# Scalsol/mega.pytorch

Measured on AMD Instinct MI355X. Metric: frames/sec MEGA R-101 inference, 1000x600 VID clip, higher is better.
Workload: dtype bf16

## Files before the change

### mega/pytorch_amd/csrc/bneck64.hip

```cpp
#include <cstdlib>

#include "common.h"

namespace {

constexpr int BK_TY = 8, BK_TX = 16;
constexpr int BK_PY = BK_TY + 2, BK_PX = BK_TX + 2;
constexpr int BK_NP = BK_PY * BK_PX;
constexpr int BK_M1 = 192;
constexpr int BK_NT = 512;
constexpr int BK_W2ROW = 1168;
constexpr int BK_WROW = 144;
constexpr int BK_SBROW = 528;
constexpr int BK_OFF_W2 = 0;
constexpr int BK_OFF_T1 = 64 * BK_W2ROW;
constexpr int BK_OFF_XB = BK_OFF_T1 + BK_NP * 128;
constexpr int BK_OFF_W1 = BK_OFF_XB + BK_M1 * 128;
constexpr int BK_XB_BYTES = 256 * BK_WROW;
constexpr int BK_OFF_T2 = BK_OFF_XB + BK_XB_BYTES;
constexpr int BK_LDS = BK_OFF_T2 + 128 * 128;
constexpr int BK_OFF_ST = BK_OFF_T1;
static_assert(BK_OFF_ST + 128 * BK_SBROW <= BK_LDS, "staging must fit");
static_assert(BK_M1 * 128 + 64 * BK_WROW <= BK_XB_BYTES, "x chunk + w1 chunk must fit the XB region");

struct Bneck64Params {
  const bf16_t* x;
  const bf16_t* w1;
  const bf16_t* w2;
  const bf16_t* w3;
  const float *s1, *b1, *s2, *b2, *s3, *b3;
  bf16_t* out;
  int N, H, W, tiles_y, tiles_x, ntiles;
};

template <typename HT>
__device__ __forceinline__ f32x16_t bk_mma(f32x16_t acc, const uint4& a, const uint4& b) {
  return Half16<HT>::mfma32(__builtin_bit_cast(u32x4_t, a), __builtin_bit_cast(u32x4_t, b), acc);
}

template <typename HT>
__device__ __forceinline__ unsigned bk_relu_pack(float a, float b) {
  const s16x2_t z = {0, 0};
  return __builtin_bit_cast(unsigned, __builtin_elementwise_max(__builtin_bit_cast(s16x2_t, Half16<HT>::pack2(a, b)), z));
}
template <typename HT>
__device__ __forceinline__ bf16_t bk_relu1(float a) {
  const bf16_t h = Half16<HT>::cvt(a);
  return (short)h < 0 ? (bf16_t)0 : h;
}

template <typename HT>
__global__ __launch_bounds__(BK_NT, 2) void bneck64_kernel(Bneck64Params p) {
  extern __shared__ __attribute__((aligned(16))) unsigned char smem[];
  unsigned char* const w2l = smem + BK_OFF_W2;
  unsigned char* const t1l = smem + BK_OFF_T1;
  unsigned char* const xbl = smem + BK_OFF_XB;
  unsigned char* const w1l = smem + BK_OFF_W1;
  unsigned char* const t2l = smem + BK_OFF_T2;
  unsigned char* const sbl = smem + BK_OFF_ST;
  const int tid = threadIdx.x, lane = tid & 63, wave = tid >> 6;
  const int l31 = lane & 31, h = lane >> 5;

  {
    const uint4* wg = reinterpret_cast<const uint4*>(p.w2);
    for (int e = tid; e < 64 * 72; e += BK_NT) {
      const int n = e / 72, c = e - n * 72;
      *reinterpret_cast<uint4*>(w2l + n * BK_W2ROW + c * 16) = wg[e];
    }
  }

  const unsigned xbytes = (unsigned)((size_t)p.N * p.H * p.W * 512);
  const __amdgpu_buffer_rsrc_t rs_x = __builtin_amdgcn_make_buffer_rsrc(const_cast<bf16_t*>(p.x), 0, (int)xbytes, 0x00020000);
  const __amdgpu_buffer_rsrc_t rs_o = __builtin_amdgcn_make_buffer_rsrc(p.out, 0, (int)xbytes, 0x00020000);
  constexpr unsigned OOB = 0x80000000u;

  auto tile_origin = [&](int t, int& n, int& y0, int& x0) {
    const int per_img = p.tiles_y * p.tiles_x;
    n = t / per_img;
    const int r = t - n * per_img;
    const int ty = r / p.tiles_x;
    y0 = ty * BK_TY;
    x0 = (r - ty * p.tiles_x) * BK_TX;
  };

  u32x4_t px[12], pw1[4];
  auto prefetch = [&](int t) {
    int n, y0, x0;
    const bool live = t < p.ntiles;
    tile_origin(live ? t : 0, n, y0, x0);
    unsigned off[3];
#pragma unroll
    for (int i = 0; i < 3; ++i) {
      const int v = tid + BK_NT * i;
      const int row = v >> 3, j = v & 7;
      const int py = row / BK_PX, pxx = row - py * BK_PX;
      const int yy = y0 - 1 + py, xx = x0 - 1 + pxx;
      const bool ok = live && row < BK_NP && (unsigned)yy < (unsigned)p.H && (unsigned)xx < (unsigned)p.W;
      off[i] = ok ? (unsigned)(((n * p.H + yy) * p.W + xx) * 512 + j * 16) : OOB;
    }
#pragma unroll
    for (int kc = 0; kc < 4; ++kc) {
#pragma unroll
      for (int i = 0; i < 3; ++i) {
        px[3 * kc + i] = __builtin_amdgcn_raw_buffer_load_b128(rs_x, off[i], kc * 128, 0);
      }
      pw1[kc] = *reinterpret_cast<const u32x4_t*>(p.w1 + (tid >> 3) * 256 + kc * 64 + (tid & 7) * 8);
    }
  };

  const int r1 = 32 * wave + l31;
  const unsigned a1_base = (unsigned)(r1 * 128), a1_sw = (unsigned)((r1 >> 1) & 7);
  const unsigned b1_base = (unsigned)(l31 * BK_WROW + h * 16);
  const int mb2 = wave >> 1, nb2 = wave & 1;
  const int ay = 2 * mb2 + (l31 >> 4), ax = l31 & 15;
  const unsigned a2_base = (unsigned)((ay * BK_PX + ax) * 128);
  const int b2_off = (32 * nb2 + l31) * BK_W2ROW + h * 16;
  const unsigned a3_base = (unsigned)(l31 * 128), a3_sw = (unsigned)((l31 >> 1) & 7);
  const unsigned b3_base = (unsigned)((32 * wave + l31) * BK_WROW + h * 16);
  const float s1a = p.s1[l31], s1b = p.s1[32 + l31], b1a = p.b1[l31], b1b = p.b1[32 + l31];
  const float s2v = p.s2[32 * nb2 + l31], b2v = p.b2[32 * nb2 + l31];
  const float s3v = p.s3[32 * wave + l31], b3v = p.b3[32 * wave + l31];

  int t = blockIdx.x;
  prefetch(t);
  __syncthreads();
  for (; t < p.ntiles; t += gridDim.x) {
    int n, y0, x0;
    tile_origin(t, n, y0, x0);
    f32x16_t c1a, c1b;
#pragma unroll
    for (int r = 0; r < 16; ++r) { c1a[r] = 0.f; c1b[r] = 0.f; }
#pragma unroll
    for (int kc = 0; kc < 4; ++kc) {
#pragma unroll
      for (int i = 0; i < 3; ++i) {
        const int v = tid + BK_NT * i;
        const int row = v >> 3, j = v & 7;
        *reinterpret_cast<u32x4_t*>(xbl + row * 128 + ((j ^ ((row >> 1) & 7)) * 16)) = px[3 * kc + i];
      }
      *reinterpret_cast<u32x4_t*>(w1l + (tid >> 3) * BK_WROW + (tid & 7) * 16) = pw1[kc];
      __syncthreads();
      if (wave < 6) {
#pragma unroll
        for (int ks = 0; ks < 4; ++ks) {
          const uint4 a = *reinterpret_cast<const uint4*>(xbl + a1_base + (((unsigned)(2 * ks + h) ^ a1_sw) << 4));
          const uint4 b0 = *reinterpret_cast<const uint4*>(w1l + b1_base + ks * 32);
          const uint4 b1 = *reinterpret_cast<const uint4*>(w1l + 32 * BK_WROW + b1_base + ks * 32);
          c1a = bk_mma<HT>(c1a, a, b0);
          c1b = bk_mma<HT>(c1b, a, b1);
        }
      }
      __syncthreads();
    }
    u32x4_t pw3[4];
#pragma unroll
    for (int i = 0; i < 4; ++i) pw3[i] = reinterpret_cast<const u32x4_t*>(p.w3)[tid + BK_NT * i];
    int ho = h, lo = l31;
    asm volatile("" : "+v"(ho), "+v"(lo));
    if (wave < 6) {
#pragma unroll
      for (int r = 0; r < 16; ++r) {
        const int R = 32 * wave + (r & 3) + 8 * (r >> 2) + 4 * ho;
        if (R < BK_NP) {
          const int py = R / BK_PX, pxx = R - py * BK_PX;
          const int yy = y0 - 1 + py, xx = x0 - 1 + pxx;
          const bool in = (unsigned)yy < (unsigned)p.H && (unsigned)xx < (unsigned)p.W;
          const bf16_t ra = bk_relu1<HT>(c1a[r] * s1a + b1a), rb = bk_relu1<HT>(c1b[r] * s1b + b1b);
          const bf16_t va = in ? ra : (bf16_t)0;
          const bf16_t vb = in ? rb : (bf16_t)0;
          unsigned char* base = t1l + R * 128;
          const int sw = (pxx >> 1) & 7;
          *reinterpret_cast<bf16_t*>(base + (((lo >> 3) ^ sw) * 16) + (lo & 7) * 2) = va;
          *reinterpret_cast<bf16_t*>(base + ((((32 + lo) >> 3) ^ sw) * 16) + (lo & 7) * 2) = vb;
        }
      }
    }
#pragma unroll
    for (int i = 0; i < 4; ++i) {
      const int v = tid + BK_NT * i;
      *reinterpret_cast<u32x4_t*>(xbl + (v >> 3) * BK_WROW + (v & 7) * 16) = pw3[i];
    }
    prefetch(t + gridDim.x);
    __syncthreads();
    f32x16_t c2;
#pragma unroll
    for (int r = 0; r < 16; ++r) c2[r] = 0.f;
#pragma unroll
    for (int kh = 0; kh < 3; ++kh)
#pragma unroll
      for (int kw = 0; kw < 3; ++kw)
#pragma unroll
        for (int ks = 0; ks < 4; ++ks) {
          const unsigned sw2 = (unsigned)(((ax + kw) >> 1) & 7);
          const uint4 a = *reinterpret_cast<const uint4*>(t1l + a2_base + (kh * BK_PX + kw) * 128 +
                                                          (((unsigned)(2 * ks + h) ^ sw2) << 4));
          const uint4 b = *reinterpret_cast<const uint4*>(w2l + b2_off + (kh * 3 + kw) * 128 + ks * 32);
          c2 = bk_mma<HT>(c2, a, b);
        }
    {
      const int c = 32 * nb2 + lo;
#pragma unroll
      for (int r = 0; r < 16; ++r) {
        const int P = 32 * mb2 + (r & 3) + 8 * (r >> 2) + 4 * ho;
        *reinterpret_cast<bf16_t*>(t2l + P * 128 + (((c >> 3) ^ ((P >> 1) & 7)) * 16) + (c & 7) * 2) = bk_relu1<HT>(c2[r] * s2v + b2v);
      }
    }
    __syncthreads();
    unsigned pk[4][8];
    {
      uint4 bf[4];
#pragma unroll
      for (int ks = 0; ks < 4; ++ks) bf[ks] = *reinterpret_cast<const uint4*>(xbl + b3_base + ks * 32);
      const int c3ch = 32 * wave + lo;
      const unsigned res_base = (unsigned)(((n * p.H + y0) * p.W + x0 + 4 * ho) * 512 + c3ch * 2);
#pragma unroll
      for (int mb = 0; mb < 4; ++mb) {
        __builtin_amdgcn_sched_barrier(0);
        float rs[16];
#pragma unroll
        for (int r = 0; r < 16; ++r) {
          const int yy = y0 + 2 * mb + (r >> 3), xx = x0 + (r & 3) + 8 * ((r >> 2) & 1) + 4 * ho;
          const unsigned o = (yy < p.H && xx < p.W) ? res_base : OOB;
          const unsigned short q = __builtin_amdgcn_raw_buffer_load_b16(
              rs_x, o, ((2 * mb + (r >> 3)) * p.W + (r & 3) + 8 * ((r >> 2) & 1)) * 512, 0);
          rs[r] = Half16<HT>::one(q);
        }
        f32x16_t c3;
#pragma unroll
        for (int r = 0; r < 16; ++r) c3[r] = 0.f;
#pragma unroll
        for (int ks = 0; ks < 4; ++ks) {
          const uint4 a = *reinterpret_cast<const uint4*>(t2l + mb * 4096 + a3_base + (((unsigned)(2 * ks + h) ^ a3_sw) << 4));
          c3 = bk_mma<HT>(c3, a, bf[ks]);
        }
#pragma unroll
        for (int q = 0; q < 8; ++q) {
          float v0 = c3[2 * q] * s3v + b3v, v1 = c3[2 * q + 1] * s3v + b3v;
          v0 += rs[2 * q];
          v1 += rs[2 * q + 1];
          pk[mb][q] = bk_relu_pack<HT>(v0, v1);
        }
      }
    }
    __syncthreads();
    {
      const int c3ch = 32 * wave + lo;
#pragma unroll
      for (int mb = 0; mb < 4; ++mb)
#pragma unroll
        for (int r = 0; r < 16; ++r) {
          const int P = 32 * mb + (r & 3) + 8 * (r >> 2) + 4 * ho;
          const unsigned v = pk[mb][r >> 1];
          *reinterpret_cast<bf16_t*>(sbl + P * BK_SBROW + c3ch * 2) = (bf16_t)((r & 1) ? (v >> 16) : (v & 0xffffu));
        }
    }
    __syncthreads();
#pragma unroll
    for (int i = 0; i < 8; ++i) {
      const int id = tid + BK_NT * i;
      const int P = id >> 5, cv = id & 31;
      const int yy = y0 + (P >> 4), xx = x0 + (P & 15);
      const uint4 v = *reinterpret_cast<const uint4*>(sbl + P * BK_SBROW + cv * 16);
      const u32x4_t q = {v.x, v.y, v.z, v.w};
      const unsigned o = (yy < p.H && xx < p.W) ? (unsigned)(((n * p.H + yy) * p.W + xx) * 512 + cv * 16) : OOB;
      __builtin_amdgcn_raw_buffer_store_b128(q, rs_o, o, 0, 0);
    }
    __syncthreads();
  }
}

constexpr int BD_OFF_W2 = 0;
constexpr int BD_OFF_T1 = 64 * BK_W2ROW;
constexpr int BD_OFF_XP = BD_OFF_T1 + BK_NP * 128;
constexpr int BD_OFF_WR = BD_OFF_XP + BK_M1 * 128;
constexpr int BD_LDS = BD_OFF_WR + 256 * BK_WROW;
static_assert(BD_OFF_T1 + 128 * BK_SBROW <= BD_LDS, "output staging must fit over t1 / x patch / weight region");

struct Bneck64DsParams {
  const bf16_t* x;
  const bf16_t* w1;
  const bf16_t* w2;
  const bf16_t* w3;
  const bf16_t* wd;
  const float *s1, *b1, *s2, *b2, *s3, *b3, *sd, *bd;
  bf16_t* out;
  int N, H, W, tiles_y, tiles_x, ntiles;
};

template <typename HT>
__global__ __launch_bounds__(BK_NT, 2) void bneck64_ds_kernel(Bneck64DsParams p) {
  extern __shared__ __attribute__((aligned(16))) unsigned char smem[];
  unsigned char* const w2l = smem + BD_OFF_W2;
  unsigned char* const t1l = smem + BD_OFF_T1;
  unsigned char* const t2l = smem + BD_OFF_T1;
  unsigned char* const xpl = smem + BD_OFF_XP;
  unsigned char* const wrl = smem + BD_OFF_WR;
  unsigned char* const sbl = smem + BD_OFF_T1;
  const int tid = threadIdx.x, lane = tid & 63, wave = tid >> 6;
  const int l31 = lane & 31, h = lane >> 5;
  {
    const uint4* wg = reinterpret_cast<const uint4*>(p.w2);
    for (int e = tid; e < 64 * 72; e += BK_NT) {
      const int n = e / 72, c = e - n * 72;
      *reinterpret_cast<uint4*>(w2l + n * BK_W2ROW + c * 16) = wg[e];
    }
  }
  const unsigned xbytes = (unsigned)((size_t)p.N * p.H * p.W * 128), obytes = (unsigned)((size_t)p.N * p.H * p.W * 512);
  const __amdgpu_buffer_rsrc_t rs_x = __builtin_amdgcn_make_buffer_rsrc(const_cast<bf16_t*>(p.x), 0, (int)xbytes, 0x00020000);
  const __amdgpu_buffer_rsrc_t rs_o = __builtin_amdgcn_make_buffer_rsrc(p.out, 0, (int)obytes, 0x00020000);
  constexpr unsigned OOB = 0x80000000u;
  auto tile_origin = [&](int t, int& n, int& y0, int& x0) {
    const int per_img = p.tiles_y * p.tiles_x;
    n = t / per_img;
    const int r = t - n * per_img;
    const int ty = r / p.tiles_x;
    y0 = ty * BK_TY;
    x0 = (r - ty * p.tiles_x) * BK_TX;
  };
  u32x4_t px[3];
  auto prefetch = [&](int t) {
    int n, y0, x0;
    const bool live = t < p.ntiles;
    tile_origin(live ? t : 0, n, y0, x0);
#pragma unroll
    for (int i = 0; i < 3; ++i) {
      const int v = tid + BK_NT * i;
      const int row = v >> 3, j = v & 7;
      const int py = row / BK_PX, pxx = row - py * BK_PX;
      const int yy = y0 - 1 + py, xx = x0 - 1 + pxx;
      const bool ok = live && row < BK_NP && (unsigned)yy < (unsigned)p.H && (unsigned)xx < (unsigned)p.W;
      px[i] = __builtin_amdgcn_raw_buffer_load_b128(rs_x, ok ? (unsigned)(((n * p.H + yy) * p.W + xx) * 128 + j * 16) : OOB, 0, 0);
    }
  };
  const int r1 = 32 * wave + l31;
  const unsigned a1_base = (unsigned)(r1 * 128), a1_sw = (unsigned)((r1 >> 1) & 7);
  const unsigned bw_base = (unsigned)(l31 * BK_WROW + h * 16);
  const int mb2 = wave >> 1, nb2 = wave & 1;
  const int ay = 2 * mb2 + (l31 >> 4), ax = l31 & 15;
  const unsigned a2_base = (unsigned)((ay * BK_PX + ax) * 128);
  const int b2_off = (32 * nb2 + l31) * BK_W2ROW + h * 16;
  const unsigned a3_base = (unsigned)(l31 * 128), a3_sw = (unsigned)((l31 >> 1) & 7);
  const float s1a = p.s1[l31], s1b = p.s1[32 + l31], b1a = p.b1[l31], b1b = p.b1[32 + l31];
  const float s2v = p.s2[32 * nb2 + l31], b2v = p.b2[32 * nb2 + l31];
  const float s3v = p.s3[32 * wave + l31], b3v = p.b3[32 * wave + l31];
  const float sdv = p.sd[32 * wave + l31], bdv = p.bd[32 * wave + l31];

  int t = blockIdx.x;
  prefetch(t);
  __syncthreads();
  for (; t < p.ntiles; t += gridDim.x) {
    int n, y0, x0;
    tile_origin(t, n, y0, x0);
    int ho = h, lo = l31;
    asm volatile("" : "+v"(ho), "+v"(lo));
#pragma unroll
    for (int i = 0; i < 3; ++i) {
      const int v = tid + BK_NT * i;
      const int row = v >> 3, j = v & 7;
      *reinterpret_cast<u32x4_t*>(xpl + row * 128 + ((j ^ ((row >> 1) & 7)) * 16)) = px[i];
    }
    *reinterpret_cast<u32x4_t*>(wrl + (tid >> 3) * BK_WROW + (tid & 7) * 16) =
        *reinterpret_cast<const u32x4_t*>(p.w1 + (tid >> 3) * 64 + (tid & 7) * 8);
    u32x4_t pwd[4];
#pragma unroll
    for (int i = 0; i < 4; ++i) pwd[i] = reinterpret_cast<const u32x4_t*>(p.wd)[tid + BK_NT * i];
    __syncthreads();
    f32x16_t c1a, c1b;
#pragma unroll
    for (int r = 0; r < 16; ++r) { c1a[r] = 0.f; c1b[r] = 0.f; }
    if (wave < 6) {
#pragma unroll
      for (int ks = 0; ks < 4; ++ks) {
        const uint4 a = *reinterpret_cast<const uint4*>(xpl + a1_base + (((unsigned)(2 * ks + h) ^ a1_sw) << 4));
        const uint4 b0 = *reinterpret_cast<const uint4*>(wrl + bw_base + ks * 32);
        const uint4 b1 = *reinterpret_cast<const uint4*>(wrl + 32 * BK_WROW + bw_base + ks * 32);
        c1a = bk_mma<HT>(c1a, a, b0);
        c1b = bk_mma<HT>(c1b, a, b1);
      }
#pragma unroll
      for (int r = 0; r < 16; ++r) {
        const int R = 32 * wave + (r & 3) + 8 * (r >> 2) + 4 * ho;
        if (R < BK_NP) {
          const int py = R / BK_PX, pxx = R - py * BK_PX;
          const int yy = y0 - 1 + py, xx = x0 - 1 + pxx;
          const bool in = (unsigned)yy < (unsigned)p.H && (unsigned)xx < (unsigned)p.W;
          const bf16_t ra = bk_relu1<HT>(c1a[r] * s1a + b1a), rb = bk_relu1<HT>(c1b[r] * s1b + b1b);
          const bf16_t va = in ? ra : (bf16_t)0;
          const bf16_t vb = in ? rb : (bf16_t)0;
          unsigned char* base = t1l + R * 128;
          const int sw = (pxx >> 1) & 7;
          *reinterpret_cast<bf16_t*>(base + (((lo >> 3) ^ sw) * 16) + (lo & 7) * 2) = va;
          *reinterpret_cast<bf16_t*>(base + ((((32 + lo) >> 3) ^ sw) * 16) + (lo & 7) * 2) = vb;
        }
      }
    }
    __syncthreads();
#pragma unroll
    for (int i = 0; i < 4; ++i) {
      const int v = tid + BK_NT * i;
      *reinterpret_cast<u32x4_t*>(wrl + (v >> 3) * BK_WROW + (v & 7) * 16) = pwd[i];
    }
    u32x4_t pw3[4];
#pragma unroll
    for (int i = 0; i < 4; ++i) pw3[i] = reinterpret_cast<const u32x4_t*>(p.w3)[tid + BK_NT * i];
    prefetch(t + gridDim.x);
    f32x16_t c2;
#pragma unroll
    for (int r = 0; r < 16; ++r) c2[r] = 0.f;
#pragma unroll
    for (int kh = 0; kh < 3; ++kh)
#pragma unroll
      for (int kw = 0; kw < 3; ++kw)
#pragma unroll
        for (int ks = 0; ks < 4; ++ks) {
          const unsigned sw2 = (unsigned)(((ax + kw) >> 1) & 7);
          const uint4 a = *reinterpret_cast<const uint4*>(t1l + a2_base + (kh * BK_PX + kw) * 128 +
                                                          (((unsigned)(2 * ks + h) ^ sw2) << 4));
          const uint4 b = *reinterpret_cast<const uint4*>(w2l + b2_off + (kh * 3 + kw) * 128 + ks * 32);
          c2 = bk_mma<HT>(c2, a, b);
        }
    __syncthreads();
    {
      const int c = 32 * nb2 + lo;
#pragma unroll
      for (int r = 0; r < 16; ++r) {
        const int P = 32 * mb2 + (r & 3) + 8 * (r >> 2) + 4 * ho;
        *reinterpret_cast<bf16_t*>(t2l + P * 128 + (((c >> 3) ^ ((P >> 1) & 7)) * 16) + (c & 7) * 2) = bk_relu1<HT>(c2[r] * s2v + b2v);
      }
    }
    unsigned pk[4][8];
    {
      uint4 bf[4];
#pragma unroll
      for (int ks = 0; ks < 4; ++ks) bf[ks] = *reinterpret_cast<const uint4*>(wrl + 32 * wave * BK_WROW + bw_base + ks * 32);
#pragma unroll
      for (int mb = 0; mb < 4; ++mb) {
        const int R = (2 * mb + (l31 >> 4) + 1) * BK_PX + (l31 & 15) + 1;
        const unsigned xa = (unsigned)(R * 128), xs = (unsigned)((R >> 1) & 7);
        f32x16_t cd;
#pragma unroll
        for (int r = 0; r < 16; ++r) cd[r] = 0.f;
#pragma unroll
        for (int ks = 0; ks < 4; ++ks) {
          const uint4 a = *reinterpret_cast<const uint4*>(xpl + xa + (((unsigned)(2 * ks + h) ^ xs) << 4));
          cd = bk_mma<HT>(cd, a, bf[ks]);
        }
#pragma unroll
        for (int q = 0; q < 8; ++q) pk[mb][q] = Half16<HT>::pack2(cd[2 * q] * sdv + bdv, cd[2 * q + 1] * sdv + bdv);
      }
    }
    __syncthreads();
#pragma unroll
    for (int i = 0; i < 4; ++i) {
      const int v = tid + BK_NT * i;
      *reinterpret_cast<u32x4_t*>(wrl + (v >> 3) * BK_WROW + (v & 7) * 16) = pw3[i];
    }
    __syncthreads();
    {
      uint4 bf[4];
#pragma unroll
      for (int ks = 0; ks < 4; ++ks) bf[ks] = *reinterpret_cast<const uint4*>(wrl + 32 * wave * BK_WROW + bw_base + ks * 32);
#pragma unroll
      for (int mb = 0; mb < 4; ++mb) {
        f32x16_t c3;
#pragma unroll
        for (int r = 0; r < 16; ++r) c3[r] = 0.f;
#pragma unroll
        for (int ks = 0; ks < 4; ++ks) {
          const uint4 a = *reinterpret_cast<const uint4*>(t2l + mb * 4096 + a3_base + (((unsigned)(2 * ks + h) ^ a3_sw) << 4));
          c3 = bk_mma<HT>(c3, a, bf[ks]);
        }
#pragma unroll
        for (int q = 0; q < 8; ++q) {
          float v0 = c3[2 * q] * s3v + b3v, v1 = c3[2 * q + 1] * s3v + b3v;
          v0 += Half16<HT>::lo(pk[mb][q]);
          v1 += Half16<HT>::hi(pk[mb][q]);
          pk[mb][q] = bk_relu_pack<HT>(v0, v1);
        }
      }
    }
    __syncthreads();
    {
      const int c3ch = 32 * wave + lo;
#pragma unroll
      for (int mb = 0; mb < 4; ++mb)
#pragma unroll
        for (int r = 0; r < 16; ++r) {
          const int P = 32 * mb + (r & 3) + 8 * (r >> 2) + 4 * ho;
          const unsigned v = pk[mb][r >> 1];
          *reinterpret_cast<bf16_t*>(sbl + P * BK_SBROW + c3ch * 2) = (bf16_t)((r & 1) ? (v >> 16) : (v & 0xffffu));
        }
    }
    __syncthreads();
#pragma unroll
    for (int i = 0; i < 8; ++i) {
      const int id = tid + BK_NT * i;
      const int P = id >> 5, cv = id & 31;
      const int yy = y0 + (P >> 4), xx = x0 + (P & 15);
      const uint4 v = *reinterpret_cast<const uint4*>(sbl + P * BK_SBROW + cv * 16);
      const u32x4_t q = {v.x, v.y, v.z, v.w};
      const unsigned o = (yy < p.H && xx < p.W) ? (unsigned)(((n * p.H + yy) * p.W + xx) * 512 + cv * 16) : OOB;
      __builtin_amdgcn_raw_buffer_store_b128(q, rs_o, o, 0, 0);
    }
    __syncthreads();
  }
}

}

extern "C" int mega_bottleneck64_fwd_dt(const void* x, const void* w1, const float* s1, const float* b1, const void* w2,
                                        const float* s2, const float* b2, const void* w3, const float* s3, const float* b3,
                                        void* out, int N, int H, int W, int dtype, void* stream) {
  mega_clear_error();
  if (dtype != MEGA_BF16 && dtype != MEGA_F16) return MEGA_ERR_ARG;
  if (!x || !w1 || !s1 || !b1 || !w2 || !s2 || !b2 || !w3 || !s3 || !b3 || !out || N <= 0 || H <= 0 || W <= 0) return MEGA_ERR_ARG;
  if ((size_t)N * H * W * 256 * 2 >= 0x7FF00000ull) return MEGA_ERR_ARG;
  Bneck64Params p;
  p.x = (const bf16_t*)x; p.w1 = (const bf16_t*)w1; p.w2 = (const bf16_t*)w2; p.w3 = (const bf16_t*)w3;
  p.s1 = s1; p.b1 = b1; p.s2 = s2; p.b2 = b2; p.s3 = s3; p.b3 = b3;
  p.out = (bf16_t*)out;
  p.N = N; p.H = H; p.W = W;
  p.tiles_y = cdiv(H, BK_TY);
  p.tiles_x = cdiv(W, BK_TX);
  const long tiles = (long)N * p.tiles_y * p.tiles_x;
  if (tiles > 0x7FFFFFFF) return MEGA_ERR_ARG;
  p.ntiles = (int)tiles;
  int cus = 256;
  {
    static int cached[64] = {0};
    int dev = 0, n = 0;
    if (hipGetDevice(&dev) != hipSuccess || dev < 0 || dev >= 64) dev = 0;
    if (!cached[dev]) {
      if (hipDeviceGetAttribute(&n, hipDeviceAttributeMultiprocessorCount, dev) == hipSuccess && n > 0) cached[dev] = n;
      else cached[dev] = 256;
    }
    cus = cached[dev];
  }
  const int grid = (int)(tiles < cus ? tiles : cus);
  if (dtype == MEGA_F16) {
    (void)hipFuncSetAttribute((const void*)bneck64_kernel<f16_t>, hipFuncAttributeMaxDynamicSharedMemorySize, BK_LDS);
    hipLaunchKernelGGL(bneck64_kernel<f16_t>, dim3(grid), dim3(BK_NT), BK_LDS, (hipStream_t)stream, p);
  } else {
    (void)hipFuncSetAttribute((const void*)bneck64_kernel<bf16_t>, hipFuncAttributeMaxDynamicSharedMemorySize, BK_LDS);
    hipLaunchKernelGGL(bneck64_kernel<bf16_t>, dim3(grid), dim3(BK_NT), BK_LDS, (hipStream_t)stream, p);
  }
  return mega_check_launch();
}

extern "C" int mega_bottleneck64_ds_fwd_dt(const void* x, const void* w1, const float* s1, const float* b1, const void* w2,
                                           const float* s2, const float* b2, const void* w3, const float* s3, const float* b3,
                                           const void* wd, const float* sd, const float* bd, void* out, int N, int H, int W,
                                           int dtype, void* stream) {
  mega_clear_error();
  if (dtype != MEGA_BF16 && dtype != MEGA_F16) return MEGA_ERR_ARG;
  if (!x || !w1 || !s1 || !b1 || !w2 || !s2 || !b2 || !w3 || !s3 || !b3 || !wd || !sd || !bd || !out || N <= 0 || H <= 0 || W <= 0)
    return MEGA_ERR_ARG;
  if ((size_t)N * H * W * 256 * 2 >= 0x7FF00000ull) return MEGA_ERR_ARG;
  Bneck64DsParams p;
  p.x = (const bf16_t*)x; p.w1 = (const bf16_t*)w1; p.w2 = (const bf16_t*)w2; p.w3 = (const bf16_t*)w3; p.wd = (const bf16_t*)wd;
  p.s1 = s1; p.b1 = b1; p.s2 = s2; p.b2 = b2; p.s3 = s3; p.b3 = b3; p.sd = sd; p.bd = bd;
  p.out = (bf16_t*)out;
  p.N = N; p.H = H; p.W = W;
  p.tiles_y = cdiv(H, BK_TY);
  p.tiles_x = cdiv(W, BK_TX);
  const long tiles = (long)N * p.tiles_y * p.tiles_x;
  if (tiles > 0x7FFFFFFF) return MEGA_ERR_ARG;
  p.ntiles = (int)tiles;
  int cus = 256;
  {
    static int cached[64] = {0};
    int dev = 0, n = 0;
    if (hipGetDevice(&dev) != hipSuccess || dev < 0 || dev >= 64) dev = 0;
    if (!cached[dev]) {
      if (hipDeviceGetAttribute(&n, hipDeviceAttributeMultiprocessorCount, dev) == hipSuccess && n > 0) cached[dev] = n;
      else cached[dev] = 256;
    }
    cus = cached[dev];
  }
  const int grid = (int)(tiles < cus ? tiles : cus);
  if (dtype == MEGA_F16) {
    (void)hipFuncSetAttribute((const void*)bneck64_ds_kernel<f16_t>, hipFuncAttributeMaxDynamicSharedMemorySize, BD_LDS);
    hipLaunchKernelGGL(bneck64_ds_kernel<f16_t>, dim3(grid), dim3(BK_NT), BD_LDS, (hipStream_t)stream, p);
  } else {
    (void)hipFuncSetAttribute((const void*)bneck64_ds_kernel<bf16_t>, hipFuncAttributeMaxDynamicSharedMemorySize, BD_LDS);
    hipLaunchKernelGGL(bneck64_ds_kernel<bf16_t>, dim3(grid), dim3(BK_NT), BD_LDS, (hipStream_t)stream, p);
  }
  return mega_check_launch();
}
```

Baseline: 918.7.

## Use LDS row table for t1 epilogue and read residual from staged x tile

Adds a small per-tile LDS table that holds the precomputed swizzled t1 row offset and boundary-valid bit for each halo row. The stage-1 epilogue then uses table lookups and a dump slot for padding rows, replacing per-element divisions, bounds checks and branches. In the non-downsample kernel, the residual values are now gathered from the x chunk already staged in LDS during the stage-1 K loop, instead of being reloaded from global memory with 16 scattered buffer loads per block. This costs extra registers for the residual (32 dwords), a little extra LDS and a table fill per tile.

```diff
diff --git a/mega/pytorch_amd/csrc/bneck64.hip b/mega/pytorch_amd/csrc/bneck64.hip
--- a/mega/pytorch_amd/csrc/bneck64.hip
+++ b/mega/pytorch_amd/csrc/bneck64.hip
@@ -18,9 +18,11 @@
 constexpr int BK_OFF_W1 = BK_OFF_XB + BK_M1 * 128;
 constexpr int BK_XB_BYTES = 256 * BK_WROW;
 constexpr int BK_OFF_T2 = BK_OFF_XB + BK_XB_BYTES;
-constexpr int BK_LDS = BK_OFF_T2 + 128 * 128;
+constexpr int BK_OFF_DUMP = BK_OFF_T2 + 128 * 128;
+constexpr int BK_OFF_TB = BK_OFF_DUMP + 128;
+constexpr int BK_LDS = BK_OFF_TB + BK_M1 * 2;
 constexpr int BK_OFF_ST = BK_OFF_T1;
-static_assert(BK_OFF_ST + 128 * BK_SBROW <= BK_LDS, "staging must fit");
+static_assert(BK_OFF_ST + 128 * BK_SBROW <= BK_OFF_DUMP, "staging must fit");
 static_assert(BK_M1 * 128 + 64 * BK_WROW <= BK_XB_BYTES, "x chunk + w1 chunk must fit the XB region");
 
 struct Bneck64Params {
@@ -49,6 +51,35 @@
   return (short)h < 0 ? (bf16_t)0 : h;
 }
 
+__device__ __forceinline__ void bk_fill_rowtab(unsigned char* tbl, int tid, int y0, int x0, int H, int W, unsigned dump16) {
+  if (tid < BK_M1) {
+    const int R = tid;
+    const int py = R / BK_PX, pxx = R - py * BK_PX;
+    const int yy = y0 - 1 + py, xx = x0 - 1 + pxx;
+    const bool in = R < BK_NP && (unsigned)yy < (unsigned)H && (unsigned)xx < (unsigned)W;
+    const unsigned off16 = R < BK_NP ? (unsigned)(R * 8 + ((pxx >> 1) & 7)) : dump16;
+    const int idx = (R & ~31) + ((R >> 2) & 1) * 16 + ((R >> 3) & 3) * 4 + (R & 3);
+    *reinterpret_cast<unsigned short*>(tbl + idx * 2) = (unsigned short)(off16 | (in ? 0x8000u : 0u));
+  }
+}
+
+template <typename HT>
+__device__ __forceinline__ void bk_t1_epilogue(unsigned char* t1l, const unsigned char* tbl, int wave, int ho, int lo,
+                                               const f32x16_t& c1a, const f32x16_t& c1b, float s1a, float b1a, float s1b, float b1b) {
+  const u32x4_t e0 = *reinterpret_cast<const u32x4_t*>(tbl + (wave * 32 + ho * 16) * 2);
+  const u32x4_t e1 = *reinterpret_cast<const u32x4_t*>(tbl + (wave * 32 + ho * 16) * 2 + 16);
+  const unsigned lanec = (unsigned)(((lo >> 3) << 4) | ((lo & 7) << 1));
+#pragma unroll
+  for (int r = 0; r < 16; ++r) {
+    const unsigned e = (r < 8 ? e0 : e1)[(r >> 1) & 3];
+    const unsigned off = ((r & 1) ? (e >> 12) & 0x7fff0u : (e << 4) & 0x7fff0u) ^ lanec;
+    const bool in = (e & ((r & 1) ? 0x80000000u : 0x8000u)) != 0;
+    const bf16_t ra = bk_relu1<HT>(c1a[r] * s1a + b1a), rb = bk_relu1<HT>(c1b[r] * s1b + b1b);
+    *reinterpret_cast<bf16_t*>(t1l + off) = in ? ra : (bf16_t)0;
+    *reinterpret_cast<bf16_t*>(t1l + (off ^ 64u)) = in ? rb : (bf16_t)0;
+  }
+}
+
 template <typename HT>
 __global__ __launch_bounds__(BK_NT, 2) void bneck64_kernel(Bneck64Params p) {
   extern __shared__ __attribute__((aligned(16))) unsigned char smem[];
@@ -58,8 +89,10 @@
   unsigned char* const w1l = smem + BK_OFF_W1;
   unsigned char* const t2l = smem + BK_OFF_T2;
   unsigned char* const sbl = smem + BK_OFF_ST;
+  unsigned char* const tbl = smem + BK_OFF_TB;
   const int tid = threadIdx.x, lane = tid & 63, wave = tid >> 6;
   const int l31 = lane & 31, h = lane >> 5;
+  const int wv = __builtin_amdgcn_readfirstlane(wave);
 
   {
     const uint4* wg = reinterpret_cast<const uint4*>(p.w2);
@@ -130,6 +163,8 @@
     f32x16_t c1a, c1b;
 #pragma unroll
     for (int r = 0; r < 16; ++r) { c1a[r] = 0.f; c1b[r] = 0.f; }
+    bk_fill_rowtab(tbl, tid, y0, x0, p.H, p.W, (unsigned)((BK_OFF_DUMP - BK_OFF_T1) >> 4));
+    unsigned res[4][8];
 #pragma unroll
     for (int kc = 0; kc < 4; ++kc) {
 #pragma unroll
@@ -150,6 +185,27 @@
           c1b = bk_mma<HT>(c1b, a, b1);
         }
       }
+      if ((wv >> 1) == kc) {
+        int hr = h, lr = l31;
+        asm volatile("" : "+v"(hr), "+v"(lr));
+        const unsigned jc = (unsigned)(4 * (wv & 1) + (lr >> 3));
+        unsigned ya[8];
+#pragma unroll
+        for (int c = 0; c < 8; ++c) ya[c] = (unsigned)(hr * 512 + (lr & 7) * 2) + ((jc ^ (unsigned)((c + 2 * hr) & 7)) << 4);
+#pragma unroll
+        for (int mb = 0; mb < 4; ++mb)
+#pragma unroll
+          for (int q = 0; q < 8; ++q) {
+            s16x2_t v;
+#pragma unroll
+            for (int e = 0; e < 2; ++e) {
+              const int r = 2 * q + e;
+              const int Rc = (2 * mb + (r >> 3) + 1) * BK_PX + (r & 3) + 8 * ((r >> 2) & 1) + 1;
+              v[e] = *reinterpret_cast<const short*>(xbl + ya[(Rc >> 1) & 7] + Rc * 128);
+            }
+            res[mb][q] = __builtin_bit_cast(unsigned, v);
+          }
+      }
       __syncthreads();
     }
     u32x4_t pw3[4];
@@ -157,24 +213,7 @@
     for (int i = 0; i < 4; ++i) pw3[i] = reinterpret_cast<const u32x4_t*>(p.w3)[tid + BK_NT * i];
     int ho = h, lo = l31;
     asm volatile("" : "+v"(ho), "+v"(lo));
-    if (wave < 6) {
-#pragma unroll
-      for (int r = 0; r < 16; ++r) {
-        const int R = 32 * wave + (r & 3) + 8 * (r >> 2) + 4 * ho;
-        if (R < BK_NP) {
-          const int py = R / BK_PX, pxx = R - py * BK_PX;
-          const int yy = y0 - 1 + py, xx = x0 - 1 + pxx;
-          const bool in = (unsigned)yy < (unsigned)p.H && (unsigned)xx < (unsigned)p.W;
-          const bf16_t ra = bk_relu1<HT>(c1a[r] * s1a + b1a), rb = bk_relu1<HT>(c1b[r] * s1b + b1b);
-          const bf16_t va = in ? ra : (bf16_t)0;
-          const bf16_t vb = in ? rb : (bf16_t)0;
-          unsigned char* base = t1l + R * 128;
-          const int sw = (pxx >> 1) & 7;
-          *reinterpret_cast<bf16_t*>(base + (((lo >> 3) ^ sw) * 16) + (lo & 7) * 2) = va;
-          *reinterpret_cast<bf16_t*>(base + ((((32 + lo) >> 3) ^ sw) * 16) + (lo & 7) * 2) = vb;
-        }
-      }
-    }
+    if (wave < 6) bk_t1_epilogue<HT>(t1l, tbl, wave, ho, lo, c1a, c1b, s1a, b1a, s1b, b1b);
 #pragma unroll
     for (int i = 0; i < 4; ++i) {
       const int v = tid + BK_NT * i;
@@ -211,20 +250,8 @@
       uint4 bf[4];
 #pragma unroll
       for (int ks = 0; ks < 4; ++ks) bf[ks] = *reinterpret_cast<const uint4*>(xbl + b3_base + ks * 32);
-      const int c3ch = 32 * wave + lo;
-      const unsigned res_base = (unsigned)(((n * p.H + y0) * p.W + x0 + 4 * ho) * 512 + c3ch * 2);
 #pragma unroll
       for (int mb = 0; mb < 4; ++mb) {
-        __builtin_amdgcn_sched_barrier(0);
-        float rs[16];
-#pragma unroll
-        for (int r = 0; r < 16; ++r) {
-          const int yy = y0 + 2 * mb + (r >> 3), xx = x0 + (r & 3) + 8 * ((r >> 2) & 1) + 4 * ho;
-          const unsigned o = (yy < p.H && xx < p.W) ? res_base : OOB;
-          const unsigned short q = __builtin_amdgcn_raw_buffer_load_b16(
-              rs_x, o, ((2 * mb + (r >> 3)) * p.W + (r & 3) + 8 * ((r >> 2) & 1)) * 512, 0);
-          rs[r] = Half16<HT>::one(q);
-        }
         f32x16_t c3;
 #pragma unroll
         for (int r = 0; r < 16; ++r) c3[r] = 0.f;
@@ -236,8 +263,8 @@
 #pragma unroll
         for (int q = 0; q < 8; ++q) {
           float v0 = c3[2 * q] * s3v + b3v, v1 = c3[2 * q + 1] * s3v + b3v;
-          v0 += rs[2 * q];
-          v1 += rs[2 * q + 1];
+          v0 += Half16<HT>::lo(res[mb][q]);
+          v1 += Half16<HT>::hi(res[mb][q]);
           pk[mb][q] = bk_relu_pack<HT>(v0, v1);
         }
       }
@@ -273,8 +300,10 @@
 constexpr int BD_OFF_T1 = 64 * BK_W2ROW;
 constexpr int BD_OFF_XP = BD_OFF_T1 + BK_NP * 128;
 constexpr int BD_OFF_WR = BD_OFF_XP + BK_M1 * 128;
-constexpr int BD_LDS = BD_OFF_WR + 256 * BK_WROW;
-static_assert(BD_OFF_T1 + 128 * BK_SBROW <= BD_LDS, "output staging must fit over t1 / x patch / weight region");
+constexpr int BD_OFF_DUMP = BD_OFF_WR + 256 * BK_WROW;
+constexpr int BD_OFF_TB = BD_OFF_DUMP + 128;
+constexpr int BD_LDS = BD_OFF_TB + BK_M1 * 2;
+static_assert(BD_OFF_T1 + 128 * BK_SBROW <= BD_OFF_DUMP, "output staging must fit over t1 / x patch / weight region");
 
 struct Bneck64DsParams {
   const bf16_t* x;
@@ -296,6 +325,7 @@
   unsigned char* const xpl = smem + BD_OFF_XP;
   unsigned char* const wrl = smem + BD_OFF_WR;
   unsigned char* const sbl = smem + BD_OFF_T1;
+  unsigned char* const tbl = smem + BD_OFF_TB;
   const int tid = threadIdx.x, lane = tid & 63, wave = tid >> 6;
   const int l31 = lane & 31, h = lane >> 5;
   {
@@ -361,6 +391,7 @@
     }
     *reinterpret_cast<u32x4_t*>(wrl + (tid >> 3) * BK_WROW + (tid & 7) * 16) =
         *reinterpret_cast<const u32x4_t*>(p.w1 + (tid >> 3) * 64 + (tid & 7) * 8);
+    bk_fill_rowtab(tbl, tid, y0, x0, p.H, p.W, (unsigned)((BD_OFF_DUMP - BD_OFF_T1) >> 4));
     u32x4_t pwd[4];
 #pragma unroll
     for (int i = 0; i < 4; ++i) pwd[i] = reinterpret_cast<const u32x4_t*>(p.wd)[tid + BK_NT * i];
@@ -377,22 +408,7 @@
         c1a = bk_mma<HT>(c1a, a, b0);
         c1b = bk_mma<HT>(c1b, a, b1);
       }
-#pragma unroll
-      for (int r = 0; r < 16; ++r) {
-        const int R = 32 * wave + (r & 3) + 8 * (r >> 2) + 4 * ho;
-        if (R < BK_NP) {
-          const int py = R / BK_PX, pxx = R - py * BK_PX;
-          const int yy = y0 - 1 + py, xx = x0 - 1 + pxx;
-          const bool in = (unsigned)yy < (unsigned)p.H && (unsigned)xx < (unsigned)p.W;
-          const bf16_t ra = bk_relu1<HT>(c1a[r] * s1a + b1a), rb = bk_relu1<HT>(c1b[r] * s1b + b1b);
-          const bf16_t va = in ? ra : (bf16_t)0;
-          const bf16_t vb = in ? rb : (bf16_t)0;
-          unsigned char* base = t1l + R * 128;
-          const int sw = (pxx >> 1) & 7;
-          *reinterpret_cast<bf16_t*>(base + (((lo >> 3) ^ sw) * 16) + (lo & 7) * 2) = va;
-          *reinterpret_cast<bf16_t*>(base + ((((32 + lo) >> 3) ^ sw) * 16) + (lo & 7) * 2) = vb;
-        }
-      }
+      bk_t1_epilogue<HT>(t1l, tbl, wave, ho, lo, c1a, c1b, s1a, b1a, s1b, b1b);
     }
     __syncthreads();
 #pragma unroll
```

After: 924.4, median of 5. About the same (+0.6%).
